# SIMPLE-BuildingSimulation/heat

Hardware: AMD Instinct MI355X
Metric: surface-node-updates/sec (higher is better)
Workload: dtype f64

## Files before the change

### heat_amd/csrc/batch.hip

```cpp
#include <hip/hip_runtime.h>
#include <rccl/rccl.h>

#include <dlfcn.h>

#include <algorithm>
#include <cmath>
#include <cstdarg>
#include <cstdio>
#include <cstdlib>
#include <cstring>
#include <limits>
#include <mutex>
#include <numeric>
#include <string>
#include <vector>

#include "batch.hpp"

namespace {

struct Rccl {
    void *handle = nullptr;
    ncclResult_t (*GetUniqueId)(ncclUniqueId *) = nullptr;
    ncclResult_t (*CommInitRank)(ncclComm_t *, int, ncclUniqueId, int) = nullptr;
// ... 77 lines not shown
        if (side[i]) (void)hipStreamDestroy(side[i]);
    }
    if (fused_stream) (void)hipStreamDestroy(fused_stream);
    if (ev_fork) (void)hipEventDestroy(ev_fork);
    if (ev_fused) (void)hipEventDestroy(ev_fused);
    if (ev_staged) (void)hipEventDestroy(ev_staged);
    if (own_stream && stream) (void)hipStreamDestroy(stream);
}

namespace {

int flags_to_status(int f) {
    if (f & FLAG_NAN_HS) return fail(HEAT_N_NAN_HS, "NaN convection coefficient (reference: surface.rs:704)");
    if (f & FLAG_NAN_NOMASS) return fail(HEAT_N_NAN_NOMASS, "NaN error in the no-mass loop (reference: surface.rs:850)");
    if (f & FLAG_NAN_ZONE) return fail(HEAT_N_NAN_ZONE, "NaN zone temperature (reference: model.rs:417)");
    if (f & FLAG_UNREACHABLE) return fail(HEAT_N_UNREACHABLE, "unreachable!() branch taken (NaN input)");
    if (f & FLAG_EXCHANGE)
        return fail(HEAT_E_DEVICE, "cluster-resident march: a workgroup of a team gave up waiting for another member's zone sums "
                                   "(the state of this march call is not to be used)");
    return HEAT_OK;
}

int rebuild_unified(heat_batch *b);

int build(heat_batch *b, const heat_batch_desc *d, const heat_batch_options &opt, int32_t n_sites = 1,
          const int32_t *site_of_surface = nullptr) {
    Plan p;
    {
        std::string err;
        const int rc = make_plan(d, opt, p, err, n_sites, site_of_surface);
        if (rc) return fail(rc, "%s", err.c_str());
    }
    b->n_sites = p.n_sites;
    if (!p.dev_site.empty()) HIP_TRY(b->d_site.upload(p.dev_site));
    b->h_site = p.dev_site;
    const int64_t S = p.n_surf, Z = p.n_zones;
    b->n_surf = S;
    b->n_zones = Z;
    b->n_state = p.n_state;
    b->n_cav = p.n_cav;
    b->dt = p.dt;
    b->n_nodes = p.n_nodes;
    b->algorithmic_bytes = p.algorithmic_bytes;
    for (int i = 0; i < 5; i++) b->class_counts[i] = p.class_counts[i];
    b->n_palette = p.n_palette;
    b->n_fused_surfaces = p.n_fused_surfaces;
    b->gen_base = p.gen_base;
    b->node_slots = p.node_slots;
    b->n_small_tiles = p.n_small_tiles;
    b->n_small_plain_tiles = p.n_small_plain_tiles;
    b->n_smallcav_stream_tiles = b->n_smallcav_stream_tiles0 = p.n_smallcav_stream_tiles;
    b->any_fused = p.any_fused;
    b->h_zone_block = p.zone_block;
    b->h_gen_tiles0 = b->h_gen_tiles_cur = p.gen_tiles;
    for (int c = 0; c < kNumFast; c++) {
        for (int g2 = 0; g2 < 4; g2++) {
            b->h_fblocks[c][g2] = b->h_fblocks0[c][g2] = p.fblocks[c][g2];
            HIP_TRY(b->d_fblocks[c][g2].upload(p.fblocks[c][g2]));
        }
        b->h_team_blocks[c] = b->h_team_blocks0[c] = p.team_blocks[c];
        b->h_team_supers[c] = p.team_supers[c];
        b->any_teams = b->any_teams || !p.team_supers[c].empty();
        HIP_TRY(b->d_team_blocks[c].upload(p.team_blocks[c]));
        HIP_TRY(b->d_team_supers[c].upload(p.team_supers[c]));
        b->h_tiles0[c] = b->h_tiles_cur[c] = p.fast_tiles[c];
        b->n_stream_tiles[c] = b->n_stream_tiles0[c] = p.n_stream_tiles[c];
        b->n_fast_tiles[c] = (int)p.fast_tiles[c].size();
        HIP_TRY(b->d_fast_tiles[c].upload(p.fast_tiles[c]));
        b->nm_count_base[c] = p.nm_count_base[c];
    }
    b->nm_count_base[kNumFast] = p.nm_count_base[kNumFast];
    b->h_fzones = p.fzones;
    HIP_TRY(b->d_fzones.upload(p.fzones));
    HIP_TRY(b->d_fzone_eoff.upload(p.fzone_eoff));
    HIP_TRY(b->d_team_zinfo.upload(p.team_zinfo));
    HIP_TRY(b->d_fslots.upload(p.fslots));
    HIP_TRY(b->d_side_area.upload(p.side_area));
    HIP_TRY(b->d_side_lzone.upload(p.side_lzone));
    b->h_touched = p.touched;
    b->h_owned = p.touched;
    if (b->n_ranks <= 1) b->h_owned.assign(Z, 1);
    {
        std::vector<int32_t> sz;
        for (int64_t z = 0; z < Z; z++) if (b->h_zone_block[z] < 0 && b->h_owned[z]) sz.push_back((int32_t)z);
        b->n_stream_zones = (int)sz.size();
        HIP_TRY(b->d_stream_zones.upload(sz));
    }

    b->h_first_slot = std::move(p.h_first_slot);
    b->h_node_count = std::move(p.h_node_count);
    for (int a = 0; a < 4; a++) b->h_out_slots[a] = std::move(p.h_out_slots[a]);
    b->h_zone_slot_h = p.zone_slot;

    b->n_gen_tiles = (int)p.gen_tiles.size();
    HIP_TRY(b->d_gen_tiles.upload(p.gen_tiles));
// ... 440 lines not shown
    const bool persist = persist_min > 0 && n_sub >= persist_min;
    const int n_cu = b->n_cu;
    if (b->d_fqueue.n == 0) HIP_TRY(b->d_fqueue.zeros(kNumFast * 4));
    for (int c = 0; c < kNumFast; c++)
        for (int g2 = 0; g2 < 4; g2++) {
            const int nb = (int)b->h_fblocks[c][g2].size();
            if (nb == 0) continue;
            fa.blocks = b->d_fblocks[c][g2].p;
            fa.n_blocks = nb;
            fa.queue = nullptr;
            int grid = nb;
            if (beside_exchange || persist) {
                const int fw = (g2 & 1) ? 8 : 4;
                static const int room_env = getenv("HEAT_AMD_FUSED_ROOM") ? atoi(getenv("HEAT_AMD_FUSED_ROOM")) : 0;
                const int room = room_env > 0 ? room_env : n_cu * fused_blocks_per_cu(kFastM[c], kFastCAV[c], g2 >> 1, fw, b->na.pal_stride, ideal);
                const int reserve = !beside_exchange ? 0 : reserve_env >= 0 ? reserve_env
                                                     : std::min(room / 2, std::max(fw == 4 ? 16 : 8, (int)(room * streamed_share)));
                if (nb > room - reserve) {
                    grid = std::max(1, room - reserve);
                    fa.queue = b->d_fqueue.p + c * 4 + g2;
                    fa.queue_base = b->fqueue_base[c * 4 + g2];
                }
            }
            static const bool trace = getenv("HEAT_AMD_TRACE") != nullptr;
            if (trace)
                fprintf(stderr, "heat_amd: fused launch%s%s: %d workgroups for %d blocks (class %d, list %d, %d sub-timesteps)\n",
                        fa.queue ? " on the work queue" : "", ideal ? " with ideal loads" : "", grid, nb, c, g2, n_sub);
            b->n_fused_launches++;
            const int nm_variant = kFastNM[c] ? ((b->class_has_chunks[c] && !(g2 >> 1) && !kFastCAV[c] && kFastM[c] <= 8) ? 2 : 1) : 0;
            HIP_TRY(launch_surfaces_fused(kFastM[c], nm_variant, kFastCAV[c], g2 >> 1, (g2 & 1) ? 8 : 4, grid, b->d_fast_tiles[c].p, b->n_fast_tiles[c],
                                          b->na, b->sa, b->d_weather.p, b->d_flags.p,
                                          b->d_nomass_iters.p + b->nm_count_base[c], fa, st, ideal));
            if (fa.queue) b->fqueue_base[c * 4 + g2] += (unsigned int)nb;
        }
    for (int c = 0; c < kNumFast; c++) {
        const int n_super = (int)b->h_team_supers[c].size();
        if (n_super == 0) continue;
        const int team_size = team_shape[c].team_size, n_teams = team_shape[c].n_teams;
        if (b->xbuf_teams < n_teams) {
            HIP_TRY(b->d_xbuf.zeros((size_t)n_teams * 2 * kTeamZones * kTeamMax * 4));
            b->xbuf_teams = n_teams;
        }
        b->team_epoch++;
        if ((b->team_epoch & 1023u) == 0) {
            HIP_TRY(hipMemsetAsync(b->d_xbuf.p, 0, b->d_xbuf.n * sizeof(unsigned long long), st));
            b->team_epoch++;
// ... 534 lines not shown
            for (FusedBlock &fb : tb) {
                const int first = (int)t.size();
                t.insert(t.end(), t0.begin() + fb.first_tile, t0.begin() + fb.first_tile + fb.n_tiles);
                fb.first_tile = first;
                n_kept_tiles += fb.n_tiles;
                for (int j = 0; j < fb.n_zones; j++) zone_fused[b->h_fzones[fb.first_zone + j]] = 1;
                for (int q = 0; q < fb.n_tiles; q++) n_fused_now += t[fb.first_tile + q].G;
            }
            b->h_team_blocks[c] = tb;
            HIP_TRY(b->d_team_blocks[c].upload(tb));
            b->any_fused = b->any_fused || !tb.empty();
        }
        for (int g2 = 0; g2 < 4; g2++) {
            for (const FusedBlock &fb : keep[g2]) {
                n_kept_tiles += fb.n_tiles;
                for (int q = 0; q < fb.n_tiles; q++) n_fused_now += t[fb.first_tile + q].G;
            }
            b->h_fblocks[c][g2] = keep[g2];
            HIP_TRY(b->d_fblocks[c][g2].upload(keep[g2]));
            b->any_fused = b->any_fused || !keep[g2].empty();
        }
        b->n_stream_tiles[c] = (int)t.size() - n_kept_tiles;
        HIP_TRY(b->d_fast_tiles[c].upload(t));
        b->h_tiles_cur[c] = t;
    }
    {
        std::vector<int32_t> szl, tz;
        for (int64_t z = 0; z < b->n_zones; z++) {
            b->h_zone_block[z] = zone_fused[z] ? 0 : -1;
            if (!zone_fused[z] && b->h_owned[z]) szl.push_back((int32_t)z);
        }
        b->n_stream_zones = (int)szl.size();
        HIP_TRY(b->d_stream_zones.upload(szl));
        for (int32_t z : zl) if (!zone_fused[z]) tz.push_back(z);
        b->n_touched_stream = (int)tz.size();
        HIP_TRY(b->d_zlist_stream.upload(tz));
    }
    b->n_fused_surfaces = n_fused_now;
    rc = rebuild_unified(b);
    if (rc) return rc;
    if (b->graph_exec) {
        HIP_TRY(hipStreamSynchronize(b->stream));
        (void)hipGraphExecDestroy(b->graph_exec);
        b->graph_exec = nullptr;
    }
    HIP_TRY(hipDeviceSynchronize());
// ... 479 lines not shown
```

### heat_amd/csrc/batch.hpp

```cpp
#pragma once
#include <hip/hip_runtime.h>
#include <rccl/rccl.h>

#include <cmath>
#include <cstdarg>
#include <cstdio>
#include <string>
#include <utility>
#include <vector>

#include "../../include/heat_amd.h"
#include "kernels.hpp"
#include "layout.hpp"
#include "hostpool.hpp"
#include "plan.hpp"

namespace heat {

inline int fail(int code, const char *fmt, ...) {
    char buf[512];
    va_list ap;
    va_start(ap, fmt);
    vsnprintf(buf, sizeof buf, fmt, ap);
    va_end(ap);
// ... 48 lines not shown

struct heat_batch {
    int device = 0;
    int n_cu = 256;
    hipStream_t stream = nullptr;
    bool own_stream = false;
    static constexpr int kSideStreams = 3;
    hipStream_t side[kSideStreams] = {nullptr, nullptr, nullptr};
    hipStream_t fused_stream = nullptr;
    hipEvent_t ev_fork = nullptr, ev_join[kSideStreams] = {nullptr, nullptr, nullptr};
    int n_ranks = 1, rank = 0;
    bool use_graph = false;

    int64_t n_surf = 0, n_zones = 0, n_state = 0, n_nodes = 0, n_cav = 0;
    double dt = 0;
    int64_t algorithmic_bytes = 0;
    int64_t class_counts[5] = {0, 0, 0, 0, 0};
    int64_t n_palette = 0;

    int64_t n_fused_surfaces = 0;
    int n_stream_tiles[kNumFast] = {};
    std::vector<FusedBlock> h_fblocks[kNumFast][4];
    DevBuf<FusedBlock> d_fblocks[kNumFast][4];
    std::vector<FusedBlock> h_team_blocks[kNumFast], h_team_blocks0[kNumFast];
    std::vector<FusedSuper> h_team_supers[kNumFast];
    DevBuf<FusedBlock> d_team_blocks[kNumFast];
    DevBuf<FusedSuper> d_team_supers[kNumFast];
    DevBuf<uint32_t> d_team_zinfo;
    DevBuf<unsigned long long> d_xbuf;
    int xbuf_teams = 0;
    uint32_t team_epoch = 0;
    bool any_teams = false;
    DevBuf<unsigned int> d_fqueue;
    unsigned int fqueue_base[kNumFast * 4] = {};
    DevBuf<int32_t> d_fzones, d_fzone_eoff;
    DevBuf<uint16_t> d_fslots;
    DevBuf<double> d_side_area;
    DevBuf<int16_t> d_side_lzone;
    std::vector<FastTile> h_tiles0[kNumFast];
    std::vector<FusedBlock> h_fblocks0[kNumFast][4];
    int n_stream_tiles0[kNumFast] = {};
    std::vector<int32_t> h_fzones;
    DevBuf<int32_t> d_zlist_stream;
    int n_touched_stream = 0;
    std::vector<int32_t> h_zone_block;
    DevBuf<int32_t> d_stream_zones;
    int n_stream_zones = 0;
    bool any_fused = false;
    hipEvent_t ev_fused = nullptr;
    hipEvent_t ev_staged = nullptr;
    bool staged = false;
    int n_fast_tiles[kNumFast] = {};
    DevBuf<FastTile> d_fast_tiles[kNumFast];
    std::vector<FastTile> h_tiles_cur[kNumFast];
    DevBuf<FastTile> d_ulist[2];
    int n_ulist[2] = {0, 0};
    int ulist_part[2][kStreamVariants][2] = {};
    bool capturing = false;
    bool host_zones_stale = false;
    unsigned int sweep_parity = 0;
    unsigned int fused_parity = 0;
    bool class_has_chunks[kNumFast] = {};
    bool in_ulist[2][kNumFast] = {};
    bool small_in_ulist[2] = {false, false};
    bool smallcav_in_ulist[2] = {false, false};
// ... 115 lines not shown
```

### heat_amd/csrc/kernels.hip

```cpp
#include <hip/hip_runtime.h>

#include <algorithm>
#include <atomic>
#include <cstdlib>

#include "device_math.hpp"
#include "kernels.hpp"
#include "layout.hpp"

namespace heat {

__device__ __forceinline__ void eval_side(const SideConst &c, const StepWeather &w, double air_t, double rad_alt,
                                          double rad_out, double surf_t, double &hs, double &rad_t, int &bad) {
    const double natural = tarp_natural(air_t, surf_t, c.cos_eff, bad);
    if ((c.kind_n & 3) == KIND_OUTDOOR) {
        const bool windward = (c.kind_n & 4) ? true : ((c.nx * w.sin_wd + c.ny * w.cos_wd) > 0.0);
        const double wf = windward ? 1.0 : 0.5;
        hs = wf * (c.forced * w.sqrt_ws) + natural;
        rad_t = rad_out;
    } else {
        hs = natural;
        rad_t = rad_alt;
    }
}
// ... 483 lines not shown
        l.zb0[threadIdx.x] = fa.b0[z];
        l.zvol[threadIdx.x] = fa.vol[z];
        if constexpr (IDEAL) fused_ideal_init(fa, l, z);
    }
    const int n_e = fa.zone_eoff[blk.first_zone + blk.n_zones] - e_first;
    for (int e = threadIdx.x; e < n_e; e += n_threads) l.slots[fa.slots[e_first + e]] = (unsigned short)e;
    __syncthreads();
}

struct FusedPre {
    int e_first, n_e, zoff, z, slot0;
    double zT, za0, zb0, zvol;
};
__device__ __forceinline__ void fused_pre_a(const FusedBlock &blk, const FusedArgs &fa, FusedPre &p) {
    p = FusedPre{0, 0, 0, 0, 0, 0.0, 0.0, 0.0, 0.0};
    const int nz = blk.n_zones;
    if (nz > 0) {
        p.e_first = fa.zone_eoff[blk.first_zone];
        p.n_e = fa.zone_eoff[blk.first_zone + nz];
        p.zoff = fa.zone_eoff[blk.first_zone + min((int)threadIdx.x, nz)];
        p.z = fa.zones[blk.first_zone + min((int)threadIdx.x, nz - 1)];
    }
}
__device__ __forceinline__ void fused_pre_b(const FusedBlock &blk, const FusedArgs &fa, FusedPre &p) {
    if (blk.n_zones > 0) {
        p.n_e -= p.e_first;
        p.zoff -= p.e_first;
        p.zT = fa.zone_T[p.z];
        p.za0 = fa.a0[p.z];
        p.zb0 = fa.b0[p.z];
        p.zvol = fa.vol[p.z];
        if (p.n_e > 0) p.slot0 = fa.slots[p.e_first + min((int)threadIdx.x, p.n_e - 1)];
    }
}
template <int IDEAL = 0>
__device__ __forceinline__ void fused_block_init(const FusedBlock &blk, const FusedArgs &fa, const FusedLds &l, int n_threads,
                                                 const FusedPre &p) {
    if ((int)threadIdx.x <= blk.n_zones) l.zoff[threadIdx.x] = p.zoff;
    if ((int)threadIdx.x < blk.n_zones) {
        l.zT[threadIdx.x] = p.zT;
        l.za0[threadIdx.x] = p.za0;
        l.zb0[threadIdx.x] = p.zb0;
        l.zvol[threadIdx.x] = p.zvol;
        if constexpr (IDEAL) fused_ideal_init(fa, l, p.z);
    }
    if ((int)threadIdx.x < p.n_e) l.slots[p.slot0] = (unsigned short)threadIdx.x;
    for (int e = threadIdx.x + n_threads; e < p.n_e; e += n_threads) l.slots[fa.slots[p.e_first + e]] = (unsigned short)e;
    __syncthreads();
}

// ... 334 lines not shown
        }                                                                                                     \
    } while (0)
#else
#define HEAT_STAMP(k, real) do { } while (0)
#define HEAT_STAMP_VALUE(k, v) do { } while (0)
#endif
#ifdef HEAT_STREAM_STAMPS
#ifndef HEAT_STAMPS
constexpr int kStampsPerBlock = 8;
__device__ unsigned long long g_stamps[65536 * kStampsPerBlock];
#endif
#define HEAT_SSTAMP(k, drain)                                                                                  \
    do {                                                                                                       \
        if constexpr (!FUSED && PAL) {                                                                         \
            if (drain) asm volatile("s_waitcnt vmcnt(0) lgkmcnt(0)" ::: "memory");                             \
            if (lane == 0 && counter_index < 32768)                                                            \
                g_stamps[(counter_index + (M == 16 ? 32768 : 0)) * kStampsPerBlock + (k)] = __builtin_amdgcn_s_memtime(); \
        }                                                                                                      \
    } while (0)
#else
#define HEAT_SSTAMP(k, drain) do { } while (0)
#endif

template <int M, int NM, int PAL, int CAV, int FUSED, int SMALL = 0, int IDEAL = 0>
__device__ __forceinline__ void fast_tile_march(const FastTile tile, int counter_index, bool nm_on, int lane, int wib,
                                                double *s_pal, double *s_V, double *s_pos, const FusedLds &fl, const FusedBlock &blk,
                                                int blk_waves, int n_it, int step0, const NodeArrays &na,
                                                const SideArrays &sd, const StepWeather *__restrict__ weather,
                                                const double *__restrict__ zone_T, int *__restrict__ flags,
                                                unsigned long long *__restrict__ nomass_iters, const FusedArgs &fa,
                                                bool write_out = true, const TeamCtx team = TeamCtx{0, 0, 0, 0, nullptr}) {
    constexpr int kLanes = (FUSED ? FUSED : 4) * kWave;
    constexpr bool kVinLds = FUSED && fused_v_in_lds(M, NM, FUSED, SMALL);
    HEAT_STAMP(4, true);
    HEAT_STAMP(0, false);
    HEAT_SSTAMP(0, false);
    double2 *const s_hT = fl.hT;
    double *const s_zT = fl.zT;
    (void)s_hT; (void)s_zT; (void)s_V; (void)s_pos; (void)nm_on; (void)blk; (void)blk_waves; (void)counter_index;
    FusedPre pre;
    (void)pre;
    if constexpr (FUSED) fused_pre_a(blk, fa, pre);
    const bool mixed = PAL && (tile.k & kTileMixedBit) != 0;
    constexpr bool kChunks = NM == 2 && PAL;
    const bool chunky = kChunks && (tile.k & kTileChunkyBit) != 0;
    const int k = tile.k & 0xff;
    const bool full = (tile.k & 0x100) != 0;
    const int G = tile.G;
    const int Lk = mixed ? k : (kWave / k) * k;
    int g = (int)(((float)lane + 0.5f) * (1.0f / (float)k));
    int seg = lane - g * k;
    bool is_last = (seg == k - 1);
    const bool in_layout = lane < Lk;
    if (mixed) {
        const unsigned int e = reinterpret_cast<const unsigned short *>(na.cls + tile.node_base + (int64_t)M * Lk)[in_layout ? lane : 0];
        g = (int)(e & 63u);
        seg = (int)((e >> 6) & 63u);
        is_last = (e & (unsigned int)kLaneLastBit) != 0;
    }
    const bool active = in_layout && (g < G);
    if (!active) g = 0;
    const int d = tile.surf_base + g;
    const int ll = in_layout ? lane : 0;

    const int S = sd.S;
// ... 36 lines not shown
        const int ubase = na.pal_ubase;
        double *sp = s_pal + wib * (kWave * pstride);
        auto load_cls_T = [&]() {
            const unsigned char *pc = na.cls + tile.node_base + (int64_t)ll * M;
            if constexpr (M == 4) {
                cw[0] = *reinterpret_cast<const unsigned int *>(pc);
            } else {
#pragma unroll
                for (int q = 0; q < M / 8; q++) {
                    const uint2 w0 = reinterpret_cast<const uint2 *>(pc)[q];
                    cw[2 * q] = w0.x;
                    cw[2 * q + 1] = w0.y;
                }
            }
            const double2 *pT = reinterpret_cast<const double2 *>(na.T + tile.node_base);
#pragma unroll
            for (int jp = 0; jp < M / 2; jp++) {
                const double2 t = pT[jp * Lk + ll];
                T[2 * jp] = t.x; T[2 * jp + 1] = t.y;
            }
        };
        if constexpr (FUSED) {
            load_cls_T();
            fused_pre_b(blk, fa, pre);
        }
        {
            const double2 *gp = reinterpret_cast<const double2 *>(na.pal + (int64_t)tile.surf_base * pstride);
            double2 *sp2 = reinterpret_cast<double2 *>(sp);
            const int n2 = G * (pstride / 2);
            for (int i0 = 0; i0 < n2; i0 += 6 * kWave) {
                double2 t6[6];
#pragma unroll
                for (int q = 0; q < 6; q++) t6[q] = gp[min(i0 + q * kWave + lane, n2 - 1)];
                if constexpr (FUSED) {
                    asm volatile("" : "+v"(t6[0].x), "+v"(t6[1].x), "+v"(t6[2].x), "+v"(t6[3].x), "+v"(t6[4].x), "+v"(t6[5].x),
                                      "+v"(pre.zT), "+v"(pre.za0), "+v"(pre.zb0), "+v"(pre.zvol), "+v"(pre.slot0));
                }
#pragma unroll
                for (int q = 0; q < 6; q++)
                    if (i0 + q * kWave + lane < n2) sp2[i0 + q * kWave + lane] = t6[q];
            }
        }
        if constexpr (!FUSED) load_cls_T();
        HEAT_STAMP(6, false);
        __builtin_amdgcn_wave_barrier();
        {
            const double *mp = sp + g * pstride;
// ... 456 lines not shown
        sd.out[sidx] = o;
    }
    if (write_out && single && active) {
        SideOut o;
        o.hs = o2_hs;
        o.flow = o2_flow;
        sd.out[S + d] = o;
    }
    if (active && bad_all) report_failure(flags, bad_all, (unsigned int)d);
#ifdef HEAT_STAMPS
    asm volatile("s_waitcnt vmcnt(0)" ::: "memory");
#endif
    HEAT_STAMP(3, false);
    HEAT_SSTAMP(3, true);
    HEAT_STAMP(5, true);
    if constexpr (NM) {
        unsigned int tot = nm_passes;
#pragma unroll
        for (int o = kWave / 2; o > 0; o >>= 1) tot += __shfl_down(tot, o, kWave);
        if (lane == 0 && tot) nomass_iters[counter_index] += tot;
    }
}

template <int M, int NM, int PAL, int CAV, int FUSED, int SMALL = 0, int IDEAL = 0>
__global__ void __launch_bounds__(FUSED ? 64 * FUSED : 256, (FUSED || (M == 16 && !CAV)) ? 2 : 1)
k_surfaces_fast(const FastTile *__restrict__ tiles, int n_tiles, NodeArrays na, SideArrays sd,
                const StepWeather *__restrict__ weather, const int *__restrict__ step_ptr, int step_fixed,
                const double *__restrict__ zone_T, int *__restrict__ flags,
                unsigned long long *__restrict__ nomass_iters, FusedArgs fa) {
    static_assert(!FUSED || (PAL && !(CAV && M == 16)),
                  "the cluster-resident march exists for palette classes; with gas cavities for 4 or 8 nodes per lane");
    static_assert(!IDEAL || (FUSED && SMALL != 2 && NM != 2 && (SMALL == 1 || !CAV)),
                  "ideal loads ride on the plain and the mixed workgroups only: no teams, no cavity class, no chunk loop");
    constexpr int kMaxW = FUSED ? FUSED : 4;
    constexpr int kLanes = kMaxW * kWave;
    extern __shared__ double s_dyn[];
    __shared__ double s_pos_static[FUSED ? 2 : kLanes];
    double *const s_pal = s_dyn;
    constexpr bool kVinLds = FUSED && fused_v_in_lds(M, NM, FUSED, SMALL);
    double *const s_V = s_dyn + kLanes * na.pal_stride;
    FusedLds fl;
    fl.hT = reinterpret_cast<double2 *>(s_V + (kVinLds ? M : 0) * kLanes);
    fl.zT = reinterpret_cast<double *>(fl.hT) + 4 * kLanes;
    fl.za0 = fl.zT + kFusedMaxZones;
    fl.zb0 = fl.za0 + kFusedMaxZones;
    fl.zvol = fl.zb0 + kFusedMaxZones;
    fl.zsa = fl.zvol + kFusedMaxZones;
    fl.zsb = fl.zsa + kFusedMaxZones;
    fl.zoff = reinterpret_cast<int *>(fl.zsb + kFusedMaxZones);
    fl.slots = reinterpret_cast<unsigned short *>(fl.zoff + kFusedMaxZones + 2);
    const int lane = threadIdx.x & (kWave - 1);
    const int wib = threadIdx.x >> 6;
    int wave0 = blockIdx.x * (blockDim.x >> 6) + wib;
    int n_waves = gridDim.x * (blockDim.x >> 6);
    FusedBlock blk{0, 0, 0, 0, 0, 0};
    int blk_waves = 0;
    int bi = blockIdx.x;
    __shared__ int s_next_block;
    const int n_it = FUSED ? fa.n_sub : 1;
    const int step0 = FUSED ? 0 : ((step_fixed >= 0) ? step_fixed : *step_ptr);
    const bool write_out = FUSED || step_fixed >= 0 || step0 == step_ptr[1];
    constexpr bool kTeam = FUSED && SMALL == 2;
    TeamCtx team{0, 0, 0, 0, flags};
    int sb = 0, n_teams = 1;
    if constexpr (kTeam) {
        team.team = (int)blockIdx.x / fa.team_size;
        team.member = (int)blockIdx.x % fa.team_size;
        n_teams = (int)gridDim.x / fa.team_size;
        sb = team.team;
    }
    for (int wave = wave0; FUSED ? (kTeam ? (sb < fa.n_super) : (bi < fa.n_blocks)) : (wave < n_tiles); wave += n_waves) {
    if constexpr (FUSED) {
        if constexpr (kTeam) {
            const FusedSuper su = fa.supers[fa.reverse ? fa.n_super - 1 - sb : sb];
            if (team.member >= su.n_members) {
                sb += n_teams;
                team.round++;
                continue;
            }
            bi = su.first_block + team.member;
        }
        blk = fa.blocks[(!kTeam && fa.reverse) ? fa.n_blocks - 1 - bi : bi];
        blk_waves = blk.n_tiles + (SMALL == 1 ? blk.n_small : 0);
        const bool looping = kTeam || fa.queue != nullptr;
        if (wib >= blk_waves) {
            if (!looping) return;
            for (int q = 0; q < kFusedBarriersAtInit; q++) __syncthreads();
            for (int it = 0; it < fa.n_sub; it++)
                for (int q = 0; q < kFusedBarriersPerSubstep; q++) __syncthreads();
            goto next_block;
        }
        if constexpr (SMALL == 1) {
            if (wib >= blk.n_tiles) {
                fused_small_wave<IDEAL>(blk, fa, fl, kLanes, wib, blk_waves, lane, na, sd, weather, flags);
                if (!looping) return;
                goto next_block;
            }
        }
        wave = blk.first_tile + wib;
    }
    {
    const int tix = (!FUSED && fa.reverse) ? n_tiles - 1 - wave : wave;
    const FastTile tl = tiles[tix];
    fast_tile_march<M, NM, PAL, CAV, FUSED, SMALL, IDEAL>(tl, tix, true, lane, wib, s_pal, s_V, s_pos_static, fl, blk, blk_waves, n_it, step0,
                                                          na, sd, site_weather(weather, sd, tl.surf_base), zone_T, flags, nomass_iters,
                                                          fa, write_out, team);
    }
next_block:
    if constexpr (FUSED) {
        if constexpr (kTeam) {
            __syncthreads();
            sb += n_teams;
            team.round++;
        } else {
            if (fa.queue == nullptr) break;
            __syncthreads();
            if (threadIdx.x == 0) s_next_block = (int)(gridDim.x + (atomicAdd(fa.queue, 1u) - fa.queue_base));
            __syncthreads();
            bi = s_next_block;
        }
    }
    }
}

constexpr int kTileKindShift = 9;
constexpr int kTileNmBit = 1 << 11;
enum { kStreamWide = 0, kStreamLight = 1, kStreamChunks = 2, kStreamCav = 3 };
template <int VARIANT>
__global__ void __launch_bounds__(256, VARIANT == kStreamLight ? 3 : 2)
// ... 1586 lines not shown
                            const StepWeather *weather, const int *step_ptr, int step_fixed, const double *zone_T,
                            int *flags, unsigned long long *nomass_iters, int n_cu, hipStream_t st, int reverse) {
    if (n_tiles <= 0) return;
    static const int per_cu_env = getenv("HEAT_AMD_STREAM_BLOCKS") ? atoi(getenv("HEAT_AMD_STREAM_BLOCKS")) : 0;
    const int per_cu = per_cu_env > 0 ? per_cu_env : (variant == kStreamLight ? 3 : 2);
    const int grid = std::min(blocks_for_waves(n_tiles), n_cu * per_cu);
#define HEAT_LAUNCH_STREAM(V)                                                                                       \
    hipLaunchKernelGGL(k_surfaces_stream<V>, dim3(grid), dim3(256), pal_lds_bytes(na), st, tiles, n_tiles, na, gen_base, sa, weather, \
                       step_ptr, step_fixed, zone_T, flags, nomass_iters, reverse)
    if (variant == kStreamWide) HEAT_LAUNCH_STREAM(kStreamWide);
    else if (variant == kStreamLight) HEAT_LAUNCH_STREAM(kStreamLight);
    else if (variant == kStreamChunks) HEAT_LAUNCH_STREAM(kStreamChunks);
    else HEAT_LAUNCH_STREAM(kStreamCav);
#undef HEAT_LAUNCH_STREAM
}

size_t fused_lds_bytes(int max_waves, int M, int pal_stride, bool v_in_lds, bool ideal = false) {
    const int v_rows = v_in_lds ? M : 0;
    return (size_t)max_waves * kWave * ((pal_stride + v_rows) * sizeof(double) + 2 * sizeof(double2)) +
           6 * kFusedMaxZones * sizeof(double) + (kFusedMaxZones + 2) * sizeof(int) + kFusedMaxEntries * sizeof(uint16_t) +
           (ideal ? kFusedIdealLdsBytes : 0);
}

template <int MM, int NN, int CC, int FW, int SM, int ID = 0>
static hipError_t launch_fused_one(int grid_blocks, const FastTile *tiles, int n_tiles, const NodeArrays &na,
                                   const SideArrays &sa, const StepWeather *weather, int *flags,
                                   unsigned long long *nomass_iters, const FusedArgs &fa, hipStream_t st) {
    const size_t lds = fused_lds_bytes(FW, MM, na.pal_stride, fused_v_in_lds(MM, NN, FW, SM), ID != 0);
    constexpr int kMaxDevices = 64;
    static std::atomic<size_t> attr_bytes[kMaxDevices];
    if (lds > 160 * 1024) return hipErrorInvalidValue;
    int dev = 0;
    if (hipGetDevice(&dev) != hipSuccess || dev < 0 || dev >= kMaxDevices) dev = kMaxDevices - 1;
    if (lds > 64 * 1024 && lds > attr_bytes[dev].load(std::memory_order_acquire)) {
        hipError_t e = hipFuncSetAttribute(reinterpret_cast<const void *>(&k_surfaces_fast<MM, NN, 1, CC, FW, SM, ID>),
                                           hipFuncAttributeMaxDynamicSharedMemorySize, (int)lds);
        if (e != hipSuccess) return e;
        if (dev != kMaxDevices - 1) attr_bytes[dev].store(lds, std::memory_order_release);
    }
    hipLaunchKernelGGL((k_surfaces_fast<MM, NN, 1, CC, FW, SM, ID>), dim3(grid_blocks), dim3(kWave * FW), lds, st, tiles,
                       n_tiles, na, sa, weather, nullptr, 0, nullptr, flags, nomass_iters, fa);
    return hipSuccess;
}

int fused_blocks_per_cu(int M, int cav, int mixed, int max_waves, int pal_stride, int ideal) {
    const int waves_per_simd = (M == 4 && !cav && !mixed) ? 3 : 2;
    const int by_regs = std::max(1, waves_per_simd * 4 / max_waves);
    const bool v_in_lds = fused_v_in_lds(M, mixed ? 1 : 0, max_waves <= 4 ? 4 : 8, mixed);
    const int by_lds = std::max<int>(1, (int)(160 * 1024 / fused_lds_bytes(max_waves, M, pal_stride, v_in_lds, ideal != 0)));
    return std::min(by_regs, by_lds);
}

template <int MM, int NN>
static int team_occupancy(size_t lds) {
    int n = 0;
    if (hipOccupancyMaxActiveBlocksPerMultiprocessor(&n, reinterpret_cast<const void *>(&k_surfaces_fast<MM, NN, 1, 0, 4, 2>),
                                                     kWave * 4, lds) != hipSuccess)
        return 0;
    return n;
}
int fused_team_blocks_per_cu(int M, int nm, int pal_stride) {
    const size_t lds = fused_lds_bytes(4, M, pal_stride, fused_v_in_lds(M, nm ? 1 : 0, 4, 2));
    if (M == 4) return nm ? team_occupancy<4, 1>(lds) : team_occupancy<4, 0>(lds);
// ... 18 lines not shown
        }
#define HEAT_FUSED_INW(MM)                                                          \
    (max_waves <= 4 ? (nm ? HEAT_FUSED_I(MM, 1, 0, 4, 0) : HEAT_FUSED_I(MM, 0, 0, 4, 0)) \
                    : (nm ? HEAT_FUSED_I(MM, 1, 0, 8, 0) : HEAT_FUSED_I(MM, 0, 0, 8, 0)))
        if (M == 4) return HEAT_FUSED_INW(4);
        if (M == 8) return HEAT_FUSED_INW(8);
        return HEAT_FUSED_INW(16);
#undef HEAT_FUSED_INW
#undef HEAT_FUSED_I
    }
#define HEAT_FUSED(MM, NN, CC, FW, SM) \
    launch_fused_one<MM, NN, CC, FW, SM>(n_blocks, tiles, n_tiles, na, sa, weather, flags, nomass_iters, fa, st)
    if (mixed == 2) {
        if (cav || max_waves > 4) return hipErrorInvalidValue;
        if (M == 4) return nm ? HEAT_FUSED(4, 1, 0, 4, 2) : HEAT_FUSED(4, 0, 0, 4, 2);
        if (M == 8) return nm ? HEAT_FUSED(8, 1, 0, 4, 2) : HEAT_FUSED(8, 0, 0, 4, 2);
        return nm ? HEAT_FUSED(16, 1, 0, 4, 2) : HEAT_FUSED(16, 0, 0, 4, 2);
    }
    if (mixed) {
        if (M == 4) return max_waves <= 4 ? HEAT_FUSED(4, 1, 1, 4, 1) : HEAT_FUSED(4, 1, 1, 8, 1);
        if (M == 8) return max_waves <= 4 ? HEAT_FUSED(8, 1, 1, 4, 1) : HEAT_FUSED(8, 1, 1, 8, 1);
        return max_waves <= 4 ? HEAT_FUSED(16, 1, 0, 4, 1) : HEAT_FUSED(16, 1, 0, 8, 1);
    }
    if (nm == 2 && !cav && M <= 8) {
        if (M == 4) return max_waves <= 4 ? HEAT_FUSED(4, 2, 0, 4, 0) : HEAT_FUSED(4, 2, 0, 8, 0);
        return max_waves <= 4 ? HEAT_FUSED(8, 2, 0, 4, 0) : HEAT_FUSED(8, 2, 0, 8, 0);
    }
#define HEAT_FUSED_NW(MM, CC)                                                    \
    (max_waves <= 4 ? (nm ? HEAT_FUSED(MM, 1, CC, 4, 0) : HEAT_FUSED(MM, 0, CC, 4, 0)) \
                    : (nm ? HEAT_FUSED(MM, 1, CC, 8, 0) : HEAT_FUSED(MM, 0, CC, 8, 0)))
    if (M == 4) return cav ? HEAT_FUSED_NW(4, 1) : HEAT_FUSED_NW(4, 0);
    if (M == 8) return cav ? HEAT_FUSED_NW(8, 1) : HEAT_FUSED_NW(8, 0);
    return HEAT_FUSED_NW(16, 0);
#undef HEAT_FUSED_NW
#undef HEAT_FUSED
}

void launch_surfaces_general(const GeneralTile *tiles, int n_tiles, const NodeArrays &na, int64_t gen_base,
                             const SideArrays &sa, const CavityDev *cavs, double *scratch,
                             const StepWeather *weather, const int *step_ptr, int step_fixed,
                             const double *zone_T, int *flags, unsigned long long *nomass_iters, hipStream_t st) {
    if (n_tiles <= 0) return;
    hipLaunchKernelGGL(k_surfaces_general, dim3(blocks_for_waves(n_tiles)), dim3(256), 0, st, tiles, n_tiles, na,
                       gen_base, sa, cavs, scratch, weather, step_ptr, step_fixed, zone_T, flags, nomass_iters);
}

void launch_surfaces_small(int with_cavities, const GeneralTile *tiles, int n_tiles, const NodeArrays &na,
                           int64_t gen_base, const SideArrays &sa, const CavityDev *cavs,
                           const StepWeather *weather, const int *step_ptr, int step_fixed, const double *zone_T,
                           int *flags, unsigned long long *nomass_iters, hipStream_t st) {
    if (n_tiles <= 0) return;
    if (with_cavities)
        hipLaunchKernelGGL(k_surfaces_small<1>, dim3(blocks_for_waves(n_tiles)), dim3(256), 0, st, tiles, n_tiles, na,
                           gen_base, sa, cavs, weather, step_ptr, step_fixed, zone_T, flags, nomass_iters);
    else
        hipLaunchKernelGGL(k_surfaces_small<0>, dim3(blocks_for_waves(n_tiles)), dim3(256), 0, st, tiles, n_tiles, na,
                           gen_base, sa, cavs, weather, step_ptr, step_fixed, zone_T, flags, nomass_iters);
// ... 273 lines not shown
```

### heat_amd/csrc/kernels.hpp

```cpp
#pragma once
#include <hip/hip_runtime.h>
#include "layout.hpp"

namespace heat {

struct SlotArrays {
    const int64_t *hs_f, *hs_b, *flow_f, *flow_b, *solar_f, *solar_b, *ir_f, *ir_b;
};

void launch_surfaces_fast(int M, int nm, int pal, int cav, double grid_share, const FastTile *tiles, int n_tiles,
                          const NodeArrays &na,
                          const SideArrays &sa, const StepWeather *weather, const int *step_ptr, int step_fixed,
                          const double *zone_T, int *flags, unsigned long long *nomass_iters, int n_cu, hipStream_t st, int reverse = 0);
constexpr int kStreamKindShift = 9;
constexpr int kStreamKindSmall = 3;
constexpr int kStreamNmBit = 1 << 11;
constexpr int kStreamVariants = 4;
void launch_surfaces_stream(int variant, const FastTile *tiles, int n_tiles, const NodeArrays &na, int64_t gen_base, const SideArrays &sa,
                            const StepWeather *weather, const int *step_ptr, int step_fixed, const double *zone_T,
                            int *flags, unsigned long long *nomass_iters, int n_cu, hipStream_t st, int reverse = 0);
int fused_blocks_per_cu(int M, int cav, int mixed, int max_waves, int pal_stride, int ideal = 0);
int fused_team_blocks_per_cu(int M, int nm, int pal_stride);
hipError_t launch_surfaces_fused(int M, int nm, int cav, int mixed, int max_waves, int grid_blocks, const FastTile *tiles, int n_tiles,
                                 const NodeArrays &na, const SideArrays &sa, const StepWeather *weather, int *flags,
                                 unsigned long long *nomass_iters, const FusedArgs &fa, hipStream_t st, int ideal = 0);
void launch_surfaces_general(const GeneralTile *tiles, int n_tiles, const NodeArrays &na, int64_t gen_base,
                             const SideArrays &sa, const CavityDev *cavs, double *scratch,
                             const StepWeather *weather, const int *step_ptr, int step_fixed,
                             const double *zone_T, int *flags, unsigned long long *nomass_iters, hipStream_t st);
void launch_surfaces_small(int with_cavities, const GeneralTile *tiles, int n_tiles, const NodeArrays &na,
                           int64_t gen_base, const SideArrays &sa, const CavityDev *cavs,
                           const StepWeather *weather, const int *step_ptr, int step_fixed, const double *zone_T,
                           int *flags, unsigned long long *nomass_iters, hipStream_t st);
void launch_zones(const int64_t *zone_off, const ZoneEntry *entries, const ZoneContrib *zc,
                  const double *a0, const double *b0, const double *zone_vol, double *zone_T, double *partial,
                  int n_zones, double dt, int *step_ptr, int *flags, int mode, const int32_t *zlist, int n_list,
                  const int32_t *slot_of, int n_shared, int rows, hipStream_t st);
void launch_zone_update_shared(const double *gathered, int n_blocks, const int32_t *shared_zone, int n_shared,
                               const double *a0, const double *b0, const double *zone_vol, double *zone_T,
                               double dt, int *flags, hipStream_t st);
void launch_zone_update(const double *gathered, int n_blocks, const double *a0, const double *b0,
                        const double *zone_vol, double *zone_T, int n_zones, double dt, int *step_ptr,
                        int *flags, hipStream_t st);
void launch_nodes_fast(int M, const FastTile *tiles, int n_tiles, double *Tbuf, const int32_t *meta,
// ... 252 lines not shown
```

### heat_amd/csrc/layout.hpp

```cpp
#pragma once
#include <stdint.h>

namespace heat {

constexpr int kWave = 64;
constexpr double kSigma = 5.670374419e-8;
constexpr double kMassThreshold = 1e-5;

enum : int { KIND_SPACE = 0, KIND_AMBIENT = 1, KIND_OUTDOOR = 2 };

enum ShadeRow : int { SH_NX, SH_NY, SH_NZ, SH_UX, SH_UY, SH_UZ, SH_VX, SH_VY, SH_VZ, SH_W, SH_H, SH_OD, SH_OG, SH_PD, SH_PG, SH_ND,
                      SH_NG, SH_FD, SH_FG, kShadeRows };

enum : int { FLAG_NAN_HS = 1, FLAG_NAN_NOMASS = 2, FLAG_NAN_ZONE = 4, FLAG_UNREACHABLE = 8,
              FLAG_EXCHANGE = 16 };

struct FastTile {
    int64_t node_base;
    int32_t surf_base;
    int16_t k;
    int16_t G;
};
constexpr int kTileMixedBit = 1 << 12;
constexpr int kTileChunkyBit = 1 << 13;
// ... 75 lines not shown

struct CavityDev {
    double thickness, height, angle, eout, ein;
    int32_t gas, pad;
};

struct StepWeather {
    double t_out;
    double sqrt_ws;
    double sin_wd, cos_wd;
};

constexpr int kFusedMaxWaves = 8;
constexpr int kFusedMaxZones = 32;
constexpr int kFusedMaxEntries = 1024;
struct FusedBlock {
    int32_t first_tile;
    int32_t n_tiles;
    int32_t first_zone;
    int32_t n_zones;
    int32_t first_small;
    int32_t n_small;
};
struct FusedArgs {
    const FusedBlock *blocks;
    const int32_t *zones;
    const int32_t *zone_eoff;
    const uint16_t *slots;
    const double *side_area;
    const int16_t *side_lzone;
    const double *a0, *b0, *vol;
    double *zone_T;
    double dt;
    int32_t n_sub;
    int32_t pad;
    unsigned int *queue;
    int32_t n_blocks;
    uint32_t queue_base;
    const GeneralTile *gen_tiles;
    int64_t gen_base;
    unsigned long long *small_iters;
    const struct FusedSuper *supers;
    const uint32_t *team_zinfo;
    unsigned long long *xbuf;
    int32_t n_super;
    uint32_t tag_base;
    int32_t team_size;
    int32_t reverse;
// ... 26 lines not shown
```

Before: 554.0 billion.

## Pack fused block metadata into contiguous per-block records for plain lists

```diff
diff --git a/heat_amd/csrc/batch.hip b/heat_amd/csrc/batch.hip
--- a/heat_amd/csrc/batch.hip
+++ b/heat_amd/csrc/batch.hip
@@ -123,6 +123,18 @@
 }
 
 int rebuild_unified(heat_batch *b);
+
+int upload_block_recs(heat_batch *b, int c, const std::vector<FastTile> &tiles) {
+    for (int g2 = 0; g2 < 2; g2++) {
+        const std::vector<FusedBlock> &fb = b->h_fblocks[c][g2];
+        std::vector<FusedBlockRec> recs(fb.size());
+        const int bad = build_fused_block_recs(fb.data(), (int)fb.size(), tiles.data(), b->h_fzones.data(), b->h_fzone_eoff.data(),
+                                               recs.data());
+        if (bad) return fail(HEAT_E_SIZE, "cluster-resident march: block %d of class %d, list %d does not fit a record", bad - 1, c, g2);
+        HIP_TRY(b->d_frecs[c][g2].upload(recs));
+    }
+    return HEAT_OK;
+}
 
 int build(heat_batch *b, const heat_batch_desc *d, const heat_batch_options &opt, int32_t n_sites = 1,
           const int32_t *site_of_surface = nullptr) {
@@ -153,6 +165,8 @@
     b->n_smallcav_stream_tiles = b->n_smallcav_stream_tiles0 = p.n_smallcav_stream_tiles;
     b->any_fused = p.any_fused;
     b->h_zone_block = p.zone_block;
+    b->h_fzones = p.fzones;
+    b->h_fzone_eoff = p.fzone_eoff;
     b->h_gen_tiles0 = b->h_gen_tiles_cur = p.gen_tiles;
     for (int c = 0; c < kNumFast; c++) {
         for (int g2 = 0; g2 < 4; g2++) {
@@ -168,10 +182,10 @@
         b->n_stream_tiles[c] = b->n_stream_tiles0[c] = p.n_stream_tiles[c];
         b->n_fast_tiles[c] = (int)p.fast_tiles[c].size();
         HIP_TRY(b->d_fast_tiles[c].upload(p.fast_tiles[c]));
+        if (const int rc = upload_block_recs(b, c, p.fast_tiles[c])) return rc;
         b->nm_count_base[c] = p.nm_count_base[c];
     }
     b->nm_count_base[kNumFast] = p.nm_count_base[kNumFast];
-    b->h_fzones = p.fzones;
     HIP_TRY(b->d_fzones.upload(p.fzones));
     HIP_TRY(b->d_fzone_eoff.upload(p.fzone_eoff));
     HIP_TRY(b->d_team_zinfo.upload(p.team_zinfo));
@@ -658,6 +672,7 @@
                     fa.queue_base = b->fqueue_base[c * 4 + g2];
                 }
             }
+            if (fused_reads_records(g2 >> 1, ideal, fa.queue != nullptr)) fa.recs = b->d_frecs[c][g2].p;
             static const bool trace = getenv("HEAT_AMD_TRACE") != nullptr;
             if (trace)
                 fprintf(stderr, "heat_amd: fused launch%s%s: %d workgroups for %d blocks (class %d, list %d, %d sub-timesteps)\n",
@@ -1238,6 +1253,7 @@
         }
         b->n_stream_tiles[c] = (int)t.size() - n_kept_tiles;
         HIP_TRY(b->d_fast_tiles[c].upload(t));
+        if (const int rc = upload_block_recs(b, c, t)) return rc;
         b->h_tiles_cur[c] = t;
     }
     {
diff --git a/heat_amd/csrc/batch.hpp b/heat_amd/csrc/batch.hpp
--- a/heat_amd/csrc/batch.hpp
+++ b/heat_amd/csrc/batch.hpp
@@ -94,6 +94,7 @@
     int n_stream_tiles[kNumFast] = {};
     std::vector<FusedBlock> h_fblocks[kNumFast][4];
     DevBuf<FusedBlock> d_fblocks[kNumFast][4];
+    DevBuf<FusedBlockRec> d_frecs[kNumFast][2];
     std::vector<FusedBlock> h_team_blocks[kNumFast], h_team_blocks0[kNumFast];
     std::vector<FusedSuper> h_team_supers[kNumFast];
     DevBuf<FusedBlock> d_team_blocks[kNumFast];
@@ -113,6 +114,7 @@
     std::vector<FusedBlock> h_fblocks0[kNumFast][4];
     int n_stream_tiles0[kNumFast] = {};
     std::vector<int32_t> h_fzones;
+    std::vector<int32_t> h_fzone_eoff;
     DevBuf<int32_t> d_zlist_stream;
     int n_touched_stream = 0;
     std::vector<int32_t> h_zone_block;
diff --git a/heat_amd/csrc/kernels.hip b/heat_amd/csrc/kernels.hip
--- a/heat_amd/csrc/kernels.hip
+++ b/heat_amd/csrc/kernels.hip
@@ -529,10 +529,18 @@
         p.z = fa.zones[blk.first_zone + min((int)threadIdx.x, nz - 1)];
     }
 }
+__device__ __forceinline__ void fused_pre_rec(const FusedBlockRec *rec, FusedPre &p, int t) {
+    p = FusedPre{rec->e_first, rec->n_e, 0, 0, 0, 0.0, 0.0, 0.0, 0.0};
+    p.zoff = rec->zoff[min(t, kFusedMaxZones)];
+    p.z = rec->zones[min(t, kFusedMaxZones - 1)];
+}
+template <bool REL = false>
 __device__ __forceinline__ void fused_pre_b(const FusedBlock &blk, const FusedArgs &fa, FusedPre &p) {
     if (blk.n_zones > 0) {
-        p.n_e -= p.e_first;
-        p.zoff -= p.e_first;
+        if constexpr (!REL) {
+            p.n_e -= p.e_first;
+            p.zoff -= p.e_first;
+        }
         p.zT = fa.zone_T[p.z];
         p.za0 = fa.a0[p.z];
         p.zb0 = fa.b0[p.z];
@@ -913,25 +921,27 @@
 #define HEAT_SSTAMP(k, drain) do { } while (0)
 #endif
 
-template <int M, int NM, int PAL, int CAV, int FUSED, int SMALL = 0, int IDEAL = 0>
+template <int M, int NM, int PAL, int CAV, int FUSED, int SMALL = 0, int IDEAL = 0, int REC = 0>
 __device__ __forceinline__ void fast_tile_march(const FastTile tile, int counter_index, bool nm_on, int lane, int wib,
                                                 double *s_pal, double *s_V, double *s_pos, const FusedLds &fl, const FusedBlock &blk,
                                                 int blk_waves, int n_it, int step0, const NodeArrays &na,
                                                 const SideArrays &sd, const StepWeather *__restrict__ weather,
                                                 const double *__restrict__ zone_T, int *__restrict__ flags,
                                                 unsigned long long *__restrict__ nomass_iters, const FusedArgs &fa,
-                                                bool write_out = true, const TeamCtx team = TeamCtx{0, 0, 0, 0, nullptr}) {
+                                                bool write_out = true, const TeamCtx team = TeamCtx{0, 0, 0, 0, nullptr},
+                                                const FusedPre &pre_rec = FusedPre{0, 0, 0, 0, 0, 0.0, 0.0, 0.0, 0.0}) {
     constexpr int kLanes = (FUSED ? FUSED : 4) * kWave;
     constexpr bool kVinLds = FUSED && fused_v_in_lds(M, NM, FUSED, SMALL);
+    constexpr bool kRec = REC != 0;
     HEAT_STAMP(4, true);
     HEAT_STAMP(0, false);
     HEAT_SSTAMP(0, false);
     double2 *const s_hT = fl.hT;
     double *const s_zT = fl.zT;
     (void)s_hT; (void)s_zT; (void)s_V; (void)s_pos; (void)nm_on; (void)blk; (void)blk_waves; (void)counter_index;
-    FusedPre pre;
+    FusedPre pre = pre_rec;
     (void)pre;
-    if constexpr (FUSED) fused_pre_a(blk, fa, pre);
+    if constexpr (FUSED && !kRec) fused_pre_a(blk, fa, pre);
     const bool mixed = PAL && (tile.k & kTileMixedBit) != 0;
     constexpr bool kChunks = NM == 2 && PAL;
     const bool chunky = kChunks && (tile.k & kTileChunkyBit) != 0;
@@ -1014,7 +1024,7 @@
         };
         if constexpr (FUSED) {
             load_cls_T();
-            fused_pre_b(blk, fa, pre);
+            fused_pre_b<kRec>(blk, fa, pre);
         }
         {
             const double2 *gp = reinterpret_cast<const double2 *>(na.pal + (int64_t)tile.surf_base * pstride);
@@ -1517,7 +1527,7 @@
     }
 }
 
-template <int M, int NM, int PAL, int CAV, int FUSED, int SMALL = 0, int IDEAL = 0>
+template <int M, int NM, int PAL, int CAV, int FUSED, int SMALL = 0, int IDEAL = 0, int REC = 0>
 __global__ void __launch_bounds__(FUSED ? 64 * FUSED : 256, (FUSED || (M == 16 && !CAV)) ? 2 : 1)
 k_surfaces_fast(const FastTile *__restrict__ tiles, int n_tiles, NodeArrays na, SideArrays sd,
                 const StepWeather *__restrict__ weather, const int *__restrict__ step_ptr, int step_fixed,
@@ -1556,6 +1566,16 @@
     const int step0 = FUSED ? 0 : ((step_fixed >= 0) ? step_fixed : *step_ptr);
     const bool write_out = FUSED || step_fixed >= 0 || step0 == step_ptr[1];
     constexpr bool kTeam = FUSED && SMALL == 2;
+    static_assert(!REC || (FUSED && SMALL == 0 && !IDEAL), "block records are read by the plain lists' kernels only");
+    constexpr bool kRec = REC != 0;
+    FastTile tl_rec{0, 0, 0, 0};
+    FusedPre pre_rec{0, 0, 0, 0, 0, 0.0, 0.0, 0.0, 0.0};
+    (void)tl_rec;
+    if constexpr (kRec) {
+        double dt_own;
+        asm volatile("s_mov_b64 %0, %1" : "=s"(dt_own) : "s"(fa.dt));
+        fa.dt = dt_own;
+    }
     TeamCtx team{0, 0, 0, 0, flags};
     int sb = 0, n_teams = 1;
     if constexpr (kTeam) {
@@ -1575,7 +1595,16 @@
             }
             bi = su.first_block + team.member;
         }
-        blk = fa.blocks[(!kTeam && fa.reverse) ? fa.n_blocks - 1 - bi : bi];
+        if constexpr (kRec) {
+            int t = (int)threadIdx.x;
+            asm volatile("" : "+v"(t));
+            const FusedBlockRec *rec = fa.recs + (fa.reverse ? fa.n_blocks - 1 - bi : bi);
+            blk = rec->blk;
+            tl_rec = rec->tiles[t >> 6];
+            fused_pre_rec(rec, pre_rec, t);
+        } else {
+            blk = fa.blocks[(!kTeam && fa.reverse) ? fa.n_blocks - 1 - bi : bi];
+        }
         blk_waves = blk.n_tiles + (SMALL == 1 ? blk.n_small : 0);
         const bool looping = kTeam || fa.queue != nullptr;
         if (wib >= blk_waves) {
@@ -1596,10 +1625,12 @@
     }
     {
     const int tix = (!FUSED && fa.reverse) ? n_tiles - 1 - wave : wave;
-    const FastTile tl = tiles[tix];
-    fast_tile_march<M, NM, PAL, CAV, FUSED, SMALL, IDEAL>(tl, tix, true, lane, wib, s_pal, s_V, s_pos_static, fl, blk, blk_waves, n_it, step0,
+    FastTile tl;
+    if constexpr (kRec) tl = tl_rec;
+    else tl = tiles[tix];
+    fast_tile_march<M, NM, PAL, CAV, FUSED, SMALL, IDEAL, REC>(tl, tix, true, lane, wib, s_pal, s_V, s_pos_static, fl, blk, blk_waves, n_it, step0,
                                                           na, sd, site_weather(weather, sd, tl.surf_base), zone_T, flags, nomass_iters,
-                                                          fa, write_out, team);
+                                                          fa, write_out, team, pre_rec);
     }
 next_block:
     if constexpr (FUSED) {
@@ -3232,7 +3263,7 @@
            (ideal ? kFusedIdealLdsBytes : 0);
 }
 
-template <int MM, int NN, int CC, int FW, int SM, int ID = 0>
+template <int MM, int NN, int CC, int FW, int SM, int ID = 0, int RC = 0>
 static hipError_t launch_fused_one(int grid_blocks, const FastTile *tiles, int n_tiles, const NodeArrays &na,
                                    const SideArrays &sa, const StepWeather *weather, int *flags,
                                    unsigned long long *nomass_iters, const FusedArgs &fa, hipStream_t st) {
@@ -3243,12 +3274,12 @@
     int dev = 0;
     if (hipGetDevice(&dev) != hipSuccess || dev < 0 || dev >= kMaxDevices) dev = kMaxDevices - 1;
     if (lds > 64 * 1024 && lds > attr_bytes[dev].load(std::memory_order_acquire)) {
-        hipError_t e = hipFuncSetAttribute(reinterpret_cast<const void *>(&k_surfaces_fast<MM, NN, 1, CC, FW, SM, ID>),
+        hipError_t e = hipFuncSetAttribute(reinterpret_cast<const void *>(&k_surfaces_fast<MM, NN, 1, CC, FW, SM, ID, RC>),
                                            hipFuncAttributeMaxDynamicSharedMemorySize, (int)lds);
         if (e != hipSuccess) return e;
         if (dev != kMaxDevices - 1) attr_bytes[dev].store(lds, std::memory_order_release);
     }
-    hipLaunchKernelGGL((k_surfaces_fast<MM, NN, 1, CC, FW, SM, ID>), dim3(grid_blocks), dim3(kWave * FW), lds, st, tiles,
+    hipLaunchKernelGGL((k_surfaces_fast<MM, NN, 1, CC, FW, SM, ID, RC>), dim3(grid_blocks), dim3(kWave * FW), lds, st, tiles,
                        n_tiles, na, sa, weather, nullptr, 0, nullptr, flags, nomass_iters, fa);
     return hipSuccess;
 }
@@ -3313,17 +3344,22 @@
         if (M == 8) return max_waves <= 4 ? HEAT_FUSED(8, 1, 1, 4, 1) : HEAT_FUSED(8, 1, 1, 8, 1);
         return max_waves <= 4 ? HEAT_FUSED(16, 1, 0, 4, 1) : HEAT_FUSED(16, 1, 0, 8, 1);
     }
+    const bool rec = fused_reads_records(mixed, ideal, fa.queue != nullptr);
+#define HEAT_FUSED_R(MM, NN, CC, FW)                                                                                       \
+    (rec ? launch_fused_one<MM, NN, CC, FW, 0, 0, 1>(n_blocks, tiles, n_tiles, na, sa, weather, flags, nomass_iters, fa, st) \
+         : HEAT_FUSED(MM, NN, CC, FW, 0))
     if (nm == 2 && !cav && M <= 8) {
-        if (M == 4) return max_waves <= 4 ? HEAT_FUSED(4, 2, 0, 4, 0) : HEAT_FUSED(4, 2, 0, 8, 0);
-        return max_waves <= 4 ? HEAT_FUSED(8, 2, 0, 4, 0) : HEAT_FUSED(8, 2, 0, 8, 0);
+        if (M == 4) return max_waves <= 4 ? HEAT_FUSED_R(4, 2, 0, 4) : HEAT_FUSED_R(4, 2, 0, 8);
+        return max_waves <= 4 ? HEAT_FUSED_R(8, 2, 0, 4) : HEAT_FUSED_R(8, 2, 0, 8);
     }
 #define HEAT_FUSED_NW(MM, CC)                                                    \
-    (max_waves <= 4 ? (nm ? HEAT_FUSED(MM, 1, CC, 4, 0) : HEAT_FUSED(MM, 0, CC, 4, 0)) \
-                    : (nm ? HEAT_FUSED(MM, 1, CC, 8, 0) : HEAT_FUSED(MM, 0, CC, 8, 0)))
+    (max_waves <= 4 ? (nm ? HEAT_FUSED_R(MM, 1, CC, 4) : HEAT_FUSED_R(MM, 0, CC, 4)) \
+                    : (nm ? HEAT_FUSED_R(MM, 1, CC, 8) : HEAT_FUSED_R(MM, 0, CC, 8)))
     if (M == 4) return cav ? HEAT_FUSED_NW(4, 1) : HEAT_FUSED_NW(4, 0);
     if (M == 8) return cav ? HEAT_FUSED_NW(8, 1) : HEAT_FUSED_NW(8, 0);
     return HEAT_FUSED_NW(16, 0);
 #undef HEAT_FUSED_NW
+#undef HEAT_FUSED_R
 #undef HEAT_FUSED
 }
 
diff --git a/heat_amd/csrc/kernels.hpp b/heat_amd/csrc/kernels.hpp
--- a/heat_amd/csrc/kernels.hpp
+++ b/heat_amd/csrc/kernels.hpp
@@ -20,6 +20,7 @@
                             const StepWeather *weather, const int *step_ptr, int step_fixed, const double *zone_T,
                             int *flags, unsigned long long *nomass_iters, int n_cu, hipStream_t st, int reverse = 0);
 int fused_blocks_per_cu(int M, int cav, int mixed, int max_waves, int pal_stride, int ideal = 0);
+inline bool fused_reads_records(int mixed, int ideal, bool queued) { return mixed == 0 && ideal == 0 && !queued; }
 int fused_team_blocks_per_cu(int M, int nm, int pal_stride);
 hipError_t launch_surfaces_fused(int M, int nm, int cav, int mixed, int max_waves, int grid_blocks, const FastTile *tiles, int n_tiles,
                                  const NodeArrays &na, const SideArrays &sa, const StepWeather *weather, int *flags,
diff --git a/heat_amd/csrc/layout.hpp b/heat_amd/csrc/layout.hpp
--- a/heat_amd/csrc/layout.hpp
+++ b/heat_amd/csrc/layout.hpp
@@ -121,8 +121,40 @@
     int32_t first_small;
     int32_t n_small;
 };
+struct alignas(64) FusedBlockRec {
+    FusedBlock blk;
+    int32_t e_first;
+    int32_t n_e;
+    FastTile tiles[kFusedMaxWaves];
+    int32_t zones[kFusedMaxZones];
+    uint16_t zoff[kFusedMaxZones + 1];
+};
+static_assert(sizeof(FusedBlockRec) == 384, "FusedBlockRec: six cache lines (DESIGN.md 4a)");
+inline int build_fused_block_recs(const FusedBlock *blocks, int n_blocks, const FastTile *tiles, const int32_t *zones,
+                                  const int32_t *zone_eoff, FusedBlockRec *out) {
+    for (int i = 0; i < n_blocks; i++) {
+        const FusedBlock &b = blocks[i];
+        FusedBlockRec r{};
+        r.blk = b;
+        if (b.n_tiles < 0 || b.n_tiles > kFusedMaxWaves || b.n_zones < 0 || b.n_zones > kFusedMaxZones) return 1 + i;
+        for (int q = 0; q < b.n_tiles; q++) r.tiles[q] = tiles[b.first_tile + q];
+        if (b.n_zones > 0) {
+            const int32_t e0 = zone_eoff[b.first_zone];
+            r.e_first = e0;
+            r.n_e = zone_eoff[b.first_zone + b.n_zones] - e0;
+            if (r.n_e < 0 || r.n_e > kFusedMaxEntries) return 1 + i;
+            for (int j = 0; j < b.n_zones; j++) r.zones[j] = zones[b.first_zone + j];
+            for (int j = 0; j <= b.n_zones; j++) r.zoff[j] = (uint16_t)(zone_eoff[b.first_zone + j] - e0);
+        }
+        out[i] = r;
+    }
+    return 0;
+}
 struct FusedArgs {
-    const FusedBlock *blocks;
+    union {
+        const FusedBlock *blocks;
+        const FusedBlockRec *recs;
+    };
     const int32_t *zones;
     const int32_t *zone_eoff;
     const uint16_t *slots;
```

New measurement: 554.0 billion (median of 4 runs). About the same (+0.0%).
